# RockingMat/Prot2Text-V2-esm3

Measured on AMD Instinct MI355X. Metric: contrastive-step samples/sec (protein-text pairs), higher is better.
Workload: dtype bf16; 1 GPU; cfg3: esm2_t36_3B + Llama-3.1-8B-Instruct (text layers 1-16), per-GPU batch 16 x 1024 residues / 16 x 128 text tokens, readout mix, InfoNCE tau=0.05, adapter fwd+bwd + clip + AdamW, train mode (dropout 0.3), segments 1; global_batch=16, parallelism=dp1 (single process, no collective), streams=text tower and encoder segments on separate HIP streams

## Files before the change

### prot2text-v2-esm3_amd/csrc/epilogue.h

```cpp
#pragma once
#include "common.h"

namespace p2t {

struct EpiParams {
    const float* bias;
    void* out;
    void* z;
    int64_t ldc;
    int64_t M;
    int N;
    int n_zero;
    int accumulate;
    float drop_p;
    float drop_scale;
    uint64_t drop_seed;
    const float* cs;
    void* q; void* k; void* v;
    int seq, nh, nkv;
    int head_dim;
    float q_scale;
    const uint8_t* row_scale = nullptr;
};

// ... 30 lines not shown
        v[c] = t.x; v[c + 1] = t.y; v[c + 2] = t.z; v[c + 3] = t.w;
    }
}
template <int W> __device__ __forceinline__ void loadW(const bf16_t* p, float (&v)[W]) {
    if constexpr (W == 8) {
        load8(p, v);
    } else {
        load4(p, v);
    }
}
template <int W> __device__ __forceinline__ void zeroW(float (&v)[W]) {
#pragma unroll
    for (int c = 0; c < W; ++c) v[c] = 0.f;
}

#define P2T_EPI_APPLY2                                                                                          \
    template <int W, bool IN = false>                                                                           \
    __device__ __forceinline__ static void apply2(const EpiParams& p, int64_t m, int n, const float (&v0)[W],   \
                                                  const float (&v1)[W], const float (&b0)[W], const float (&b1)[W]) { \
        group<W, IN>(p, m, n, v0, b0);                                                                          \
        group<W, IN>(p, m, n + 32, v1, b1);                                                                     \
    }

template <typename Tout> constexpr int kStoreOps8 = (int)(8 * sizeof(Tout) / 16);

template <typename Tout>
struct EpiStore {
    static constexpr bool kRmw = false;
    static constexpr int kMinOps = 2 * kStoreOps8<Tout>;
    template <int W, bool IN = false>
    __device__ __forceinline__ static void group(const EpiParams& p, int64_t m, int n, const float (&v)[W], const float (&b)[W]) {
        Tout* o = (Tout*)p.out + m * p.ldc + n;
        float r[W];
        if (IN || n < p.N) {
#pragma unroll
            for (int j = 0; j < W; ++j) r[j] = v[j] + b[j];
            storeW<W>(o, r);
        } else if (n < p.n_zero) {
            zeroW<W>(r);
            storeW<W>(o, r);
        }
    }
    P2T_EPI_APPLY2
};

template <typename Tout, bool EXTRA = false>
struct EpiGelu {
    static constexpr bool kRmw = false;
    static constexpr int kMinOps = 2 * kStoreOps8<Tout>;
    template <int W, bool IN = false>
    __device__ __forceinline__ static void group(const EpiParams& p, int64_t m, int n, const float (&v)[W], const float (&b)[W]) {
        Tout* o = (Tout*)p.out + m * p.ldc + n;
        float zv[W], r[W];
        if (IN || n < p.N) {
#pragma unroll
            for (int j = 0; j < W; ++j) {
                zv[j] = v[j] + b[j];
                r[j] = gelu_erf_for<Tout>(zv[j]);
                if constexpr (EXTRA) {
                    if (p.drop_p > 0.f) r[j] = dropout_keep(p.drop_seed, m * (int64_t)p.N + n + j, p.drop_p) ? r[j] * p.drop_scale : 0.f;
                }
            }
            if constexpr (EXTRA) {
                if (p.z) storeW<W>((Tout*)p.z + m * p.ldc + n, zv);
            }
            storeW<W>(o, r);
        } else if (n < p.n_zero) {
            zeroW<W>(r);
            storeW<W>(o, r);
            if constexpr (EXTRA) {
                if (p.z) storeW<W>((Tout*)p.z + m * p.ldc + n, r);
            }
        }
    }
    P2T_EPI_APPLY2
};

__device__ __forceinline__ unsigned epi_pack_fp8x4(float a, float b, float c, float d) {
    int r = 0;
    r = __builtin_amdgcn_cvt_pk_fp8_f32(a, b, r, false);
    r = __builtin_amdgcn_cvt_pk_fp8_f32(c, d, r, true);
    return (unsigned)r;
}
struct EpiGeluFp8 {
    static constexpr bool kRmw = false;
    static constexpr int kMinOps = 2;
    template <int W, bool IN = false>
    __device__ __forceinline__ static void group(const EpiParams& p, int64_t m, int n, const float (&v)[W], const float (&b)[W]) {
        static_assert(W == 8, "fp8 output: MFMA kernels only (8 consecutive columns per lane)");
        uint8_t* o = (uint8_t*)p.out + m * p.ldc + n;
// ... 81 lines not shown
#pragma unroll
            for (int j = 0; j < W; ++j) r[j] += v[j];
        } else {
#pragma unroll
            for (int j = 0; j < W; ++j) r[j] = v[j];
        }
        storeW<W>(o, r);
    }
    P2T_EPI_APPLY2
};

template <typename Tout>
struct EpiSwiglu {
    static constexpr bool kRmw = false;
    static constexpr int kMinOps = kStoreOps8<Tout>;
    template <int W, bool IN = false>
    __device__ __forceinline__ static void apply2(const EpiParams& p, int64_t m, int n, const float (&g)[W], const float (&u)[W],
                                                  const float (&b0)[W], const float (&b1)[W]) {
        const int f = (n >> 6) * 32 + (n & 31);
        Tout* o = (Tout*)p.out + m * p.ldc + f;
        float r[W];
        if (IN || n < p.N) {
#pragma unroll
            for (int j = 0; j < W; ++j) r[j] = silu_for<Tout>(g[j]) * u[j];
            storeW<W>(o, r);
        } else if (f < p.n_zero) {
            zeroW<W>(r);
            storeW<W>(o, r);
        }
    }
};

template <typename Tout>
struct EpiQkvRope {
    static constexpr bool kRmw = false;
    static constexpr int kMinOps = 2 * kStoreOps8<Tout>;
    static constexpr bool kFetch = true;
    __device__ __forceinline__ static bool fetch_shared(const EpiParams& p) { return p.head_dim == 64; }
    template <int W, bool UNI = false>
    __device__ __forceinline__ static void fetch2(const EpiParams& p, int64_t m, int n, float (&c)[W], float (&s)[W]) {
        const int hd = p.head_dim, half = hd >> 1;
        const int blk = UNI ? __builtin_amdgcn_readfirstlane(n >> 6) : n >> 6;
        const int head = hd == 64 ? blk : blk >> 1;
        const int j = (hd == 64 ? 0 : 32 * (blk & 1)) + (n & 31);
        const uint32_t mu = (uint32_t)m, sq = (uint32_t)p.seq;
        const uint32_t b = mu / sq, t = mu - b * sq;
        if (UNI || head < p.nh + p.nkv) {
            loadW<W>(p.cs + (size_t)(t * (uint32_t)hd) + j, c);
            loadW<W>(p.cs + (size_t)(t * (uint32_t)hd) + half + j, s);
        }
    }
    template <int W, bool UNI = false>
    __device__ __forceinline__ static void apply2_fetched(const EpiParams& p, int64_t m, int n, const float (&v0)[W], const float (&v1)[W],
                                                          const float (&b0)[W], const float (&b1)[W], const float (&c)[W], const float (&s)[W]) {
        const int hd = p.head_dim, half = hd >> 1;
        const int blk = UNI ? __builtin_amdgcn_readfirstlane(n >> 6) : n >> 6;
        const int head = hd == 64 ? blk : blk >> 1;
        const int j = (hd == 64 ? 0 : 32 * (blk & 1)) + (n & 31);
        const uint32_t mu = (uint32_t)m, sq = (uint32_t)p.seq;
        const uint32_t b = mu / sq, t = mu - b * sq;
        float x1[W], x2[W];
#pragma unroll
        for (int e = 0; e < W; ++e) { x1[e] = v0[e] + b0[e]; x2[e] = v1[e] + b1[e]; }
        Tout* dst;
        if (head < p.nh + p.nkv) {
            const bool is_q = head < p.nh;
            const float sc = is_q ? p.q_scale : 1.0f;
            float o1[W], o2[W];
#pragma unroll
            for (int e = 0; e < W; ++e) {
                const float a1 = x1[e] * sc, a2 = x2[e] * sc;
                o1[e] = a1 * c[e] - a2 * s[e];
                o2[e] = a2 * c[e] + a1 * s[e];
            }
            dst = is_q ? (Tout*)p.q + (size_t)((b * (uint32_t)p.nh + (uint32_t)head) * sq + t) * (size_t)hd
                       : (Tout*)p.k + (size_t)((b * (uint32_t)p.nkv + (uint32_t)(head - p.nh)) * sq + t) * (size_t)hd;
            storeW<W>(dst + j, o1);
            storeW<W>(dst + half + j, o2);
        } else {
            dst = (Tout*)p.v + (size_t)((b * (uint32_t)p.nkv + (uint32_t)(head - p.nh - p.nkv)) * sq + t) * (size_t)hd;
            storeW<W>(dst + j, x1);
            storeW<W>(dst + half + j, x2);
        }
    }
    template <int W, bool IN = false>
    __device__ __forceinline__ static void apply2(const EpiParams& p, int64_t m, int n, const float (&v0)[W], const float (&v1)[W],
                                                  const float (&b0)[W], const float (&b1)[W]) {
        if (!IN && n >= p.N) return;
        float c[W], s[W];
#pragma unroll
        for (int e = 0; e < W; ++e) c[e] = s[e] = 0.f;
        fetch2<W>(p, m, n, c, s);
        apply2_fetched<W>(p, m, n, v0, v1, b0, b1, c, s);
    }
};

}
// ... 1 lines not shown
```

### prot2text-v2-esm3_amd/csrc/gemm_tile_common.h

```cpp
#pragma once
#include "common.h"
#include <type_traits>

#include "epilogue.h"

namespace p2t {

struct SplitFix {
    float* slab;
    unsigned* flag;
    unsigned* timeout;
    unsigned epoch;
};
enum { TILE_FULL = 0, TILE_PRODUCE = 1, TILE_CONSUME = 2 };


__device__ __forceinline__ void tile_coords(int id, int n_items, int tiles_m, int tiles_n, int& tm, int& tn) {
    const int q8 = n_items >> 3, r8 = n_items & 7, xcd = id & 7;
    const int swz_id = (xcd < r8 ? xcd * (q8 + 1) : r8 * (q8 + 1) + (xcd - r8) * q8) + (id >> 3);
    constexpr int GM = 4;
    const int band = swz_id / (GM * tiles_n), first_m = band * GM;
    const int gm = min(GM, tiles_m - first_m);
    const int in_band = swz_id - band * GM * tiles_n;
    tm = first_m + in_band % gm;
// ... 41 lines not shown
                v0[4] += p1.x + poison; v0[5] += p1.y + poison; v0[6] += p1.z + poison; v0[7] += p1.w + poison;
                v1[0] += p2.x + poison; v1[1] += p2.y + poison; v1[2] += p2.z + poison; v1[3] += p2.w + poison;
                v1[4] += p3.x + poison; v1[5] += p3.y + poison; v1[6] += p3.z + poison; v1[7] += p3.w + poison;
            }
            Epi::template apply2<8, INTERIOR>(ep, m, nb, v0, v1, b0, b1);
        }
    }
}

template <typename Epi, typename = void> struct epi_has_fetch_shared : std::false_type {};
template <typename Epi> struct epi_has_fetch_shared<Epi, std::void_t<decltype(&Epi::fetch_shared)>> : std::true_type {};
template <typename Epi, typename = void> struct epi_has_fetch : std::false_type {};
template <typename Epi> struct epi_has_fetch<Epi, std::void_t<decltype(Epi::kFetch)>> : std::true_type {};
#define P2T_EPI_PIN_GROUP(h, j) \
    asm volatile("" : "+a"(acc[h][0][j]), "+a"(acc[h][1][j]), "+a"(acc[h][2][j]), "+a"(acc[h][3][j])::"memory");
template <int MT, typename Epi, int P = 4>
__device__ __forceinline__ void tile_epilogue_pair(f32x4 (&acc)[2][4][MT], const EpiParams& ep, int64_t m0, int n0, int wm, int wn, int fr, int kg) {
    const int nb0 = n0 + wn * 128 + kg * 8;
    float b[2][2][8];
#pragma unroll
    for (int h = 0; h < 2; ++h)
#pragma unroll
        for (int e = 0; e < 8; ++e) b[h][0][e] = b[h][1][e] = 0.f;
    if (ep.bias) {
#pragma unroll
        for (int h = 0; h < 2; ++h) {
            loadW<8>(ep.bias + nb0 + h * 64, b[h][0]);
            loadW<8>(ep.bias + nb0 + h * 64 + 32, b[h][1]);
        }
    }
    const int64_t mrow = m0 + wm * MT * 16 + fr;
    if constexpr (epi_has_fetch_shared<Epi>::value && P > 0) {
// ... 8 lines not shown
            for (int u = 0; u < PS; ++u) Epi::template fetch2<8, true>(ep, mrow + u * 16, nb0, r[u][0], r[u][1]);
            __builtin_amdgcn_sched_barrier(0);
#pragma unroll
            for (int u = 0; u < MT; ++u) {
                float s0[8], s1[8];
#pragma unroll
                for (int e = 0; e < 8; ++e) { s0[e] = r[u % PS][0][e]; s1[e] = r[u % PS][1][e]; }
                __builtin_amdgcn_sched_barrier(0);
                if (u + PS < MT) Epi::template fetch2<8, true>(ep, mrow + (u + PS) * 16, nb0, r[u % PS][0], r[u % PS][1]);
                __builtin_amdgcn_sched_barrier(0);
#pragma unroll
                for (int h = 0; h < 2; ++h) {
                    P2T_EPI_PIN_GROUP(h, u)
                    const float v0[8] = {acc[h][0][u][0], acc[h][0][u][1], acc[h][0][u][2], acc[h][0][u][3], acc[h][1][u][0], acc[h][1][u][1], acc[h][1][u][2], acc[h][1][u][3]};
                    const float v1[8] = {acc[h][2][u][0], acc[h][2][u][1], acc[h][2][u][2], acc[h][2][u][3], acc[h][3][u][0], acc[h][3][u][1], acc[h][3][u][2], acc[h][3][u][3]};
                    Epi::template apply2_fetched<8, true>(ep, mrow + u * 16, nb0 + h * 64, v0, v1, b[h][0], b[h][1], s0, s1);
                    __builtin_amdgcn_sched_barrier(0);
                }
            }
            return;
        }
    }
    if constexpr ((Epi::kRmw || epi_has_fetch<Epi>::value) && P > 0) {
        constexpr int G = 2 * MT;
        float r[P][2][8];
        if constexpr (!Epi::kRmw) {
#pragma unroll
            for (int g = 0; g < P; ++g)
#pragma unroll
                for (int e = 0; e < 8; ++e) r[g][0][e] = r[g][1][e] = 0.f;
        }
// ... 11 lines not shown
            for (int e = 0; e < 8; ++e) { s0[e] = r[g % P][0][e]; s1[e] = r[g % P][1][e]; }
            __builtin_amdgcn_sched_barrier(0);
            if (g + P < G) Epi::template fetch2<8, true>(ep, mrow + ((g + P) % MT) * 16, nb0 + ((g + P) / MT) * 64, r[g % P][0], r[g % P][1]);
            __builtin_amdgcn_sched_barrier(0);
            Epi::template apply2_fetched<8, true>(ep, mrow + j * 16, nb0 + h * 64, v0, v1, b[h][0], b[h][1], s0, s1);
            __builtin_amdgcn_sched_barrier(0);
        }
    } else {
#pragma unroll
        for (int h = 0; h < 2; ++h)
#pragma unroll
            for (int j = 0; j < MT; ++j) {
                P2T_EPI_PIN_GROUP(h, j)
                const float v0[8] = {acc[h][0][j][0], acc[h][0][j][1], acc[h][0][j][2], acc[h][0][j][3], acc[h][1][j][0], acc[h][1][j][1], acc[h][1][j][2], acc[h][1][j][3]};
                const float v1[8] = {acc[h][2][j][0], acc[h][2][j][1], acc[h][2][j][2], acc[h][2][j][3], acc[h][3][j][0], acc[h][3][j][1], acc[h][3][j][2], acc[h][3][j][3]};
                Epi::template apply2<8, true>(ep, mrow + j * 16, nb0 + h * 64, v0, v1, b[h][0], b[h][1]);
                __builtin_amdgcn_sched_barrier(0);
            }
    }
}

}
```

### prot2text-v2-esm3_amd/csrc/gemm_w4.hip

```cpp
#include <type_traits>

#include "common.h"
#include "epilogue.h"
#include "gemm_tile_common.h"
#include "kernels.h"

namespace p2t {
#ifdef P2T_LAB
__device__ uint64_t* g_lab_stamp_ptr = nullptr;
#endif

typedef __bf16 bf16x8 __attribute__((ext_vector_type(8)));

template <typename Epi, bool PERSIST, int SCHED = 1, bool PAIRS_ONLY = false>
__global__ void __launch_bounds__(256)
    gemm_nt_w4_kernel(const bf16_t* __restrict__ A, int64_t lda, const bf16_t* __restrict__ W, int64_t ldw, int64_t M, int N, int K,
                      int tiles_m, int tiles_n, int n_items, int n_tail, int n_cover, EpiParams ep, SplitFix fix) {
    constexpr int MT = 8, NT = 8, BUF = 512 * 128, WOFF = 256 * 128, NL = 16;
#ifndef P2T_LAB
    static_assert(SCHED == 1, "the product library carries one instruction order of the K loop; order 0 is in the lab build");
#endif
    constexpr int kEpiOps = 2 * MT * Epi::kMinOps;
    constexpr int kIssuedBeforeWait = SCHED == 0 ? 6 : 9;
    constexpr int kExtCount = kIssuedBeforeWait + kEpiOps > 63 ? 63 : kIssuedBeforeWait + kEpiOps;
    __shared__ __attribute__((aligned(16))) char smem[2 * BUF];

    const int lane = threadIdx.x & 63;
    const int w = __builtin_amdgcn_readfirstlane(threadIdx.x >> 6);
    const int wm = w >> 1, wn = w & 1;
    const int nk = K >> 6;

    int item = blockIdx.x;
    int tm, tn;
    const int n_order = n_items + n_tail;
    tile_coords(item, n_order, tiles_m, tiles_n, tm, tn);
    int64_t m0 = (int64_t)tm * 256;
    int n0 = tn * 256;

    const char* a_ptr = (const char*)(A + m0 * lda);
// ... 34 lines not shown
        asm volatile("s_mov_b32 m0, %2\n\ts_nop 0\n\tglobal_load_lds_dwordx4 %0, %1" ::"v"(vo), "s"(sb), "s"(lds) : "memory");
    };
    auto mm_dma = [&](auto first, f32x4& c, const bf16x8& a, const bf16x8& b, int piece, int buf) {
        const char* sb = piece < 8 ? a_ptr : w_ptr;
        const uint32_t vo = piece < 8 ? a_voff[piece & 7] : w_voff[piece & 7];
        const uint32_t lds = lds0 + buf * BUF + (piece < 8 ? 0 : WOFF) + (w * 8 + (piece & 7)) * 1024;
        if constexpr (decltype(first)::value)
            asm volatile("s_mov_b32 m0, %5\n\tv_mfma_f32_16x16x32_bf16 %0, %1, %2, 0\n\tglobal_load_lds_dwordx4 %3, %4"
                         : "=a"(c) : "v"(a), "v"(b), "v"(vo), "s"(sb), "s"(lds) : "memory");
        else
            asm volatile("s_mov_b32 m0, %5\n\tv_mfma_f32_16x16x32_bf16 %0, %1, %2, %0\n\tglobal_load_lds_dwordx4 %3, %4"
                         : "+a"(c) : "v"(a), "v"(b), "v"(vo), "s"(sb), "s"(lds) : "memory");
    };
    using T = std::true_type;
    using F = std::false_type;
    auto stage = [&](f32x4 (&acc)[2][4][MT], auto bufc, auto first, auto rt, bool ext, bool more) {
        constexpr int B = decltype(bufc)::value;
        constexpr bool RT = decltype(rt)::value;
        using FI = decltype(first);
        const uint32_t xs1 = (x_addr + B * BUF) ^ 64u, ws1 = (w_addr + B * BUF) ^ 64u;
        const uint32_t xs0 = x_addr + (B ^ 1) * BUF, ws0 = w_addr + (B ^ 1) * BUF;
#define P2T_W4_PAIR(FF, WF, XF, P)                                                                            \
        mm(FF{}, acc[(((P) & 3) * 2) >> 2][(((P) & 3) * 2) & 3][(P) >> 2], WF[((P) & 3) * 2], XF[(P) >> 2]);   \
        mm(FF{}, acc[(((P) & 3) * 2 + 1) >> 2][(((P) & 3) * 2 + 1) & 3][(P) >> 2], WF[((P) & 3) * 2 + 1], XF[(P) >> 2]);
#define P2T_W4_R1W(I) rd(wb[I], ws1, std::integral_constant<int, (I) * 2048>{});
#define P2T_W4_R1X(J) rd(xb[J], xs1, std::integral_constant<int, (J) * 2048>{});
#define P2T_W4_R0W(I) rd(wa[I], ws0, std::integral_constant<int, (I) * 2048>{});
#define P2T_W4_R0X(J) rd(xa[J], xs0, std::integral_constant<int, (J) * 2048>{});
#define P2T_W4_G(Q) if (!RT || more) dma1(Q, B);
#define P2T_W4_GPAIR(Q, FF, WF, XF, P)                                                                                           \
        if constexpr (!RT) {                                                                                                     \
            mm_dma(FF{}, acc[(((P) & 3) * 2) >> 2][(((P) & 3) * 2) & 3][(P) >> 2], WF[((P) & 3) * 2], XF[(P) >> 2], Q, B);       \
            mm(FF{}, acc[(((P) & 3) * 2 + 1) >> 2][(((P) & 3) * 2 + 1) & 3][(P) >> 2], WF[((P) & 3) * 2 + 1], XF[(P) >> 2]);     \
        } else {                                                                                                                 \
            P2T_W4_G(Q) P2T_W4_PAIR(FF, WF, XF, P)                                                                               \
        }
#define P2T_W4_WAIT_NEXT_STAGE                                                                                                  \
        if (RT && !more) asm volatile("s_waitcnt vmcnt(0)\n\ts_barrier" ::: "memory");                                          \
        else if (FI::value && ext) asm volatile("s_waitcnt vmcnt(%0)\n\ts_barrier" ::"n"(kExtCount) : "memory");                 \
        else asm volatile("s_waitcnt vmcnt(%0)\n\ts_barrier" ::"n"(kIssuedBeforeWait) : "memory");
        if constexpr (SCHED == 1) {
            P2T_W4_R1W(0) P2T_W4_R1W(1) P2T_W4_PAIR(FI, wa, xa, 0) P2T_W4_R1X(0) P2T_W4_R1W(2) P2T_W4_PAIR(FI, wa, xa, 1) P2T_W4_R1W(3) P2T_W4_R1X(1) P2T_W4_PAIR(FI, wa, xa, 2) P2T_W4_R1W(4) P2T_W4_R1W(5) P2T_W4_PAIR(FI, wa, xa, 3)
            P2T_W4_R1X(2) P2T_W4_R1W(6) P2T_W4_PAIR(FI, wa, xa, 4) P2T_W4_R1W(7) P2T_W4_R1X(3) P2T_W4_PAIR(FI, wa, xa, 5) P2T_W4_R1X(4) P2T_W4_R1X(5) P2T_W4_PAIR(FI, wa, xa, 6) P2T_W4_R1X(6) P2T_W4_R1X(7) P2T_W4_PAIR(FI, wa, xa, 7)
            P2T_W4_PAIR(FI, wa, xa, 8) P2T_W4_PAIR(FI, wa, xa, 9) P2T_W4_PAIR(FI, wa, xa, 10)
            asm volatile("s_waitcnt lgkmcnt(0)\n\ts_barrier" ::: "memory");
            P2T_W4_GPAIR(0, FI, wa, xa, 11)
            P2T_W4_PAIR(FI, wa, xa, 12) P2T_W4_PAIR(FI, wa, xa, 13) P2T_W4_GPAIR(1, FI, wa, xa, 14) P2T_W4_PAIR(FI, wa, xa, 15)
            P2T_W4_PAIR(FI, wa, xa, 16) P2T_W4_GPAIR(2, FI, wa, xa, 17) P2T_W4_PAIR(FI, wa, xa, 18) P2T_W4_PAIR(FI, wa, xa, 19)
            P2T_W4_GPAIR(3, FI, wa, xa, 20) P2T_W4_PAIR(FI, wa, xa, 21) P2T_W4_PAIR(FI, wa, xa, 22) P2T_W4_GPAIR(4, FI, wa, xa, 23)
            P2T_W4_PAIR(FI, wa, xa, 24) P2T_W4_PAIR(FI, wa, xa, 25) P2T_W4_GPAIR(5, FI, wa, xa, 26) P2T_W4_PAIR(FI, wa, xa, 27)
            P2T_W4_PAIR(FI, wa, xa, 28) P2T_W4_GPAIR(6, FI, wa, xa, 29) P2T_W4_PAIR(FI, wa, xa, 30) P2T_W4_PAIR(FI, wa, xa, 31)
            P2T_W4_GPAIR(7, F, wb, xb, 0) P2T_W4_PAIR(F, wb, xb, 1) P2T_W4_PAIR(F, wb, xb, 2) P2T_W4_GPAIR(8, F, wb, xb, 3)
            P2T_W4_WAIT_NEXT_STAGE
            P2T_W4_R0W(0) P2T_W4_PAIR(F, wb, xb, 4) P2T_W4_R0W(1) P2T_W4_PAIR(F, wb, xb, 5) P2T_W4_R0X(0) P2T_W4_GPAIR(9, F, wb, xb, 6) P2T_W4_R0W(2) P2T_W4_PAIR(F, wb, xb, 7)
            P2T_W4_R0W(3) P2T_W4_PAIR(F, wb, xb, 8) P2T_W4_R0X(1) P2T_W4_GPAIR(10, F, wb, xb, 9) P2T_W4_R0W(4) P2T_W4_PAIR(F, wb, xb, 10) P2T_W4_R0W(5) P2T_W4_PAIR(F, wb, xb, 11)
            P2T_W4_R0X(2) P2T_W4_GPAIR(11, F, wb, xb, 12) P2T_W4_R0W(6) P2T_W4_PAIR(F, wb, xb, 13) P2T_W4_R0W(7) P2T_W4_PAIR(F, wb, xb, 14) P2T_W4_R0X(3) P2T_W4_GPAIR(12, F, wb, xb, 15)
            P2T_W4_R0X(4) P2T_W4_PAIR(F, wb, xb, 16) P2T_W4_R0X(5) P2T_W4_PAIR(F, wb, xb, 17) P2T_W4_R0X(6) P2T_W4_GPAIR(13, F, wb, xb, 18) P2T_W4_R0X(7) P2T_W4_PAIR(F, wb, xb, 19)
            P2T_W4_PAIR(F, wb, xb, 20) P2T_W4_GPAIR(14, F, wb, xb, 21) P2T_W4_PAIR(F, wb, xb, 22) P2T_W4_PAIR(F, wb, xb, 23)
            P2T_W4_GPAIR(15, F, wb, xb, 24) P2T_W4_PAIR(F, wb, xb, 25) P2T_W4_PAIR(F, wb, xb, 26) P2T_W4_PAIR(F, wb, xb, 27)
// ... 18 lines not shown
            P2T_W4_R0X(4) P2T_W4_GPAIR(10, F, wb, xb, 16) P2T_W4_R0X(5) P2T_W4_PAIR(F, wb, xb, 17) P2T_W4_R0X(6) P2T_W4_PAIR(F, wb, xb, 18) P2T_W4_R0X(7) P2T_W4_GPAIR(11, F, wb, xb, 19)
            P2T_W4_PAIR(F, wb, xb, 20) P2T_W4_PAIR(F, wb, xb, 21) P2T_W4_GPAIR(12, F, wb, xb, 22) P2T_W4_PAIR(F, wb, xb, 23)
            P2T_W4_PAIR(F, wb, xb, 24) P2T_W4_GPAIR(13, F, wb, xb, 25) P2T_W4_PAIR(F, wb, xb, 26) P2T_W4_PAIR(F, wb, xb, 27)
            P2T_W4_GPAIR(14, F, wb, xb, 28) P2T_W4_PAIR(F, wb, xb, 29) P2T_W4_PAIR(F, wb, xb, 30) P2T_W4_GPAIR(15, F, wb, xb, 31)
        }
#endif
        a_ptr += 128; w_ptr += 128;
#undef P2T_W4_WAIT_NEXT_STAGE
#undef P2T_W4_PAIR
#undef P2T_W4_R1W
#undef P2T_W4_R1X
#undef P2T_W4_R0W
#undef P2T_W4_R0X
#undef P2T_W4_G
#undef P2T_W4_GPAIR
        asm volatile("s_waitcnt lgkmcnt(0)" ::: "memory");
    };
    using I0 = std::integral_constant<int, 0>;
    using I1 = std::integral_constant<int, 1>;

    auto prologue = [&]() {
#pragma unroll
    for (int b = 0; b < 2; ++b) {
#pragma unroll
        for (int q = 0; q < NL; ++q) dma1(q, b);
        a_ptr += 128; w_ptr += 128;
    }
    asm volatile("s_waitcnt vmcnt(%0)\n\ts_barrier" ::"n"(NL) : "memory");
    rd(wa[0], w_addr, std::integral_constant<int, 0>{}); rd(wa[1], w_addr, std::integral_constant<int, 2048>{});
    rd(wa[2], w_addr, std::integral_constant<int, 4096>{}); rd(wa[3], w_addr, std::integral_constant<int, 6144>{});
    rd(wa[4], w_addr, std::integral_constant<int, 8192>{}); rd(wa[5], w_addr, std::integral_constant<int, 10240>{});
    rd(wa[6], w_addr, std::integral_constant<int, 12288>{}); rd(wa[7], w_addr, std::integral_constant<int, 14336>{});
    rd(xa[0], x_addr, std::integral_constant<int, 0>{}); rd(xa[1], x_addr, std::integral_constant<int, 2048>{});
    rd(xa[2], x_addr, std::integral_constant<int, 4096>{}); rd(xa[3], x_addr, std::integral_constant<int, 6144>{});
    rd(xa[4], x_addr, std::integral_constant<int, 8192>{}); rd(xa[5], x_addr, std::integral_constant<int, 10240>{});
    rd(xa[6], x_addr, std::integral_constant<int, 12288>{}); rd(xa[7], x_addr, std::integral_constant<int, 14336>{});
    asm volatile("s_waitcnt lgkmcnt(0)" ::: "memory");
    };
    auto k_loop = [&](f32x4 (&acc)[2][4][MT], int nk_l, bool ext, bool has_next, int64_t nm0, int nn0) {
        stage(acc, I0{}, T{}, F{}, ext, true);
        stage(acc, I1{}, F{}, F{}, false, true);
        for (int s = 2; s + 2 < nk_l; s += 2) {
            stage(acc, I0{}, F{}, F{}, false, true);
            stage(acc, I1{}, F{}, F{}, false, true);
        }
        if (has_next) {
            a_ptr = (const char*)(A + nm0 * lda);
            w_ptr = (const char*)(W + (int64_t)nn0 * ldw);
        }
        stage(acc, I0{}, F{}, T{}, false, has_next);
        stage(acc, I1{}, F{}, T{}, false, has_next);
        asm volatile("s_nop 7\n\ts_nop 7\n\ts_nop 7" ::: "memory");
#pragma unroll
        for (int h = 0; h < 2; ++h)
#pragma unroll
            for (int i = 0; i < 4; ++i)
#pragma unroll
                for (int j = 0; j < MT; ++j) asm volatile("" : "+a"(acc[h][i][j]));
    };
    if constexpr (!PAIRS_ONLY) {
    prologue();
    {
        f32x4 acc[2][4][MT];
        bool ext = false;
#ifdef P2T_LAB
        constexpr bool kDiagEpi = std::is_same<Epi, EpiStore<bf16_t>>::value || std::is_same<Epi, EpiGelu<bf16_t, false>>::value || std::is_same<Epi, EpiResid>::value;
        uint64_t* dbgp = kDiagEpi ? (uint64_t*)ep.z : nullptr;
        if (!dbgp) dbgp = g_lab_stamp_ptr;
        const bool diag = PERSIST && dbgp != nullptr;
        uint64_t d_loop = 0, d_epi = 0, d_gap = 0, d_tiles = 0, d_real = 0, t_end = 0;
        auto now = [&]() -> uint64_t { uint64_t t; asm volatile("s_memtime %0\n\ts_waitcnt lgkmcnt(0)" : "=s"(t)::"memory"); return t; };
        auto now_real = [&]() -> uint64_t { uint64_t t; asm volatile("s_memrealtime %0\n\ts_waitcnt lgkmcnt(0)" : "=s"(t)::"memory"); return t; };
#endif
        for (;;) {
            const int nxt = item + (int)gridDim.x;
            const bool has_next = PERSIST && nxt < n_items;
            int64_t nm0 = 0;
            int nn0 = 0;
            if (has_next) {
                tile_coords(nxt, n_order, tiles_m, tiles_n, tm, tn);
                nm0 = (int64_t)tm * 256;
                nn0 = tn * 256;
            }
#ifdef P2T_LAB
            uint64_t t0 = 0, r0 = 0, t1 = 0;
            if (diag) { t0 = now(); r0 = now_real(); if (ext) d_gap += t0 - t_end; }
#endif
            k_loop(acc, nk, ext, has_next, nm0, nn0);
#ifdef P2T_LAB
            if (diag) { t1 = now(); d_loop += t1 - t0; d_real += now_real() - r0; d_tiles += 1; }
#endif
            if (PERSIST) {
                int fr_e = fr, kg_e = kg;
                asm volatile("" : "+v"(fr_e), "+v"(kg_e));
                tile_epilogue_pair<MT, Epi, (epi_has_fetch<Epi>::value && !Epi::kRmw) ? 2 : 4>(acc, ep, m0, n0, wm, wn, fr_e, kg_e);
            } else {
                const bool interior = m0 + 256 <= M && n0 + 256 <= N && n0 + 256 <= n_cover;
                if (interior) {
                    tile_epilogue<MT, Epi, true>(acc[0], ep, M, N, n_cover, m0, n0, wm, 2 * wn, fr, kg);
                    tile_epilogue<MT, Epi, true>(acc[1], ep, M, N, n_cover, m0, n0, wm, 2 * wn + 1, fr, kg);
                } else {
                    tile_epilogue<MT, Epi, false>(acc[0], ep, M, N, n_cover, m0, n0, wm, 2 * wn, fr, kg);
                    tile_epilogue<MT, Epi, false>(acc[1], ep, M, N, n_cover, m0, n0, wm, 2 * wn + 1, fr, kg);
                }
            }
#ifdef P2T_LAB
            if (diag) {
                t_end = now();
                d_epi += t_end - t1;
                if (!has_next && threadIdx.x == 0) {
                    uint64_t* d = dbgp + (size_t)blockIdx.x * 8;
                    d[0] = d_loop; d[1] = d_epi; d[2] = d_gap; d[3] = d_tiles; d[4] = d_real;
                }
            }
#endif
            if (!has_next) break;
            ext = true;
            item = nxt;
            m0 = nm0;
            n0 = nn0;
        }
    }
    }
    if (PERSIST && (int)blockIdx.x < 2 * n_tail) {
        const bool producer = (int)blockIdx.x < n_tail;
        const int t = producer ? (int)blockIdx.x : (int)blockIdx.x - n_tail;
        const int nk0 = (nk >> 1) & ~1;
        tile_coords(n_items + t, n_order, tiles_m, tiles_n, tm, tn);
        m0 = (int64_t)tm * 256;
        n0 = tn * 256;
        a_ptr = (const char*)(A + m0 * lda + (producer ? nk0 * 64 : 0));
        w_ptr = (const char*)(W + (int64_t)n0 * ldw + (producer ? nk0 * 64 : 0));
        asm volatile("s_waitcnt vmcnt(0) lgkmcnt(0)\n\ts_barrier" ::: "memory");
        prologue();
        f32x4 acc2[2][4][MT];
        k_loop(acc2, producer ? nk - nk0 : nk0, false, false, 0, 0);
        if (producer) {
            float4* slab = reinterpret_cast<float4*>(fix.slab) + (int64_t)t * (64 * 256) + threadIdx.x;
#pragma unroll
            for (int h = 0; h < 2; ++h)
#pragma unroll
                for (int i = 0; i < 4; ++i)
#pragma unroll
                    for (int j = 0; j < MT; ++j)
                        slab[((h * 4 + i) * MT + j) * 256] = make_float4(acc2[h][i][j][0], acc2[h][i][j][1], acc2[h][i][j][2], acc2[h][i][j][3]);
            asm volatile("s_waitcnt vmcnt(0)" ::: "memory");
            __syncthreads();
            if (w == 0) {
                __builtin_amdgcn_fence(__ATOMIC_RELEASE, "agent");
                asm volatile("s_waitcnt vmcnt(0)" ::: "memory");
                __hip_atomic_store(fix.flag + t, fix.epoch, __ATOMIC_RELAXED, __HIP_MEMORY_SCOPE_AGENT);
// ... 41 lines not shown
    return P2T_OK;
}

template <typename Epi>
int launch_gemm_w4_persist(const void* A, int64_t lda, const void* W, int64_t ldw, int64_t M, int N, int K, int n_items, int n_tail, int grid,
                           const EpiParams& ep, const SplitFix& fix, hipStream_t s, int sched) {
    const dim3 g((unsigned)(grid < n_items ? grid : n_items));
#ifdef P2T_LAB
    if (sched == 0) {
        gemm_nt_w4_kernel<Epi, true, 0><<<g, 256, 0, s>>>((const bf16_t*)A, lda, (const bf16_t*)W, ldw, M, N, K, (int)(M / 256), N / 256, n_items, n_tail, N, ep, fix);
        P2T_LAUNCH_CHECK();
        return P2T_OK;
    }
#endif
    P2T_REQUIRE(sched == 1, "gemm (four-wave): instruction order %d is not in this build", sched);
    gemm_nt_w4_kernel<Epi, true, 1><<<g, 256, 0, s>>>((const bf16_t*)A, lda, (const bf16_t*)W, ldw, M, N, K, (int)(M / 256), N / 256, n_items, n_tail, N, ep, fix);
    P2T_LAUNCH_CHECK();
    return P2T_OK;
}
template <typename Epi>
int launch_gemm_w4_pairs(const void* A, int64_t lda, const void* W, int64_t ldw, int64_t M, int N, int K, int n_tail, const EpiParams& ep,
                         const SplitFix& fix, hipStream_t s) {
    gemm_nt_w4_kernel<Epi, true, 1, true><<<dim3((unsigned)(2 * n_tail)), 256, 0, s>>>((const bf16_t*)A, lda, (const bf16_t*)W, ldw, M, N, K, (int)(M / 256),
                                                                                      N / 256, 0, n_tail, N, ep, fix);
    P2T_LAUNCH_CHECK();
    return P2T_OK;
}
template int launch_gemm_w4_pairs<EpiResid>(const void*, int64_t, const void*, int64_t, int64_t, int, int, int, const EpiParams&, const SplitFix&, hipStream_t);
template int launch_gemm_w4_pairs<EpiStore<bf16_t>>(const void*, int64_t, const void*, int64_t, int64_t, int, int, int, const EpiParams&, const SplitFix&, hipStream_t);
template int launch_gemm_w4_pairs<EpiStore<float>>(const void*, int64_t, const void*, int64_t, int64_t, int, int, int, const EpiParams&, const SplitFix&, hipStream_t);
// ... 10 lines not shown
    if (K % 128 != 0 || K < 256 || M < 1 || (int64_t)256 * (lda > ldw ? lda : ldw) * 2 >= (int64_t)1 << 32) return P2T_ERR_UNSUPPORTED;
    const bool ob = out_dtype == P2T_BF16;
    switch (epilogue) {
        case P2T_EPI_STORE: return ob ? launch_w4<EpiStore<bf16_t>>(A, lda, W, ldw, M, N, K, n_cover, ep, s) : launch_w4<EpiStore<float>>(A, lda, W, ldw, M, N, K, n_cover, ep, s);
        case P2T_EPI_GELU: if (ob) return launch_w4<EpiGelu<bf16_t>>(A, lda, W, ldw, M, N, K, n_cover, ep, s); break;
        case P2T_EPI_RESID: return launch_w4<EpiResid>(A, lda, W, ldw, M, N, K, n_cover, ep, s);
        case P2T_EPI_QKV_ROPE: if (ob) return launch_w4<EpiQkvRope<bf16_t>>(A, lda, W, ldw, M, N, K, n_cover, ep, s); break;
        default: break;
    }
    return P2T_ERR_UNSUPPORTED;
}

}

#ifdef P2T_LAB
extern "C" int p2t_lab_set_stamp_buffer(void* ptr) {
    uint64_t* p = (uint64_t*)ptr;
    return (int)hipMemcpyToSymbol(HIP_SYMBOL(p2t::g_lab_stamp_ptr), &p, sizeof(p));
}
#endif
```

Before: 172.4 samples/s.

## Defer half of persistent w4 GEMM epilogue stores into next tile's k-loop

In the persistent four-wave GEMM, the second half of each tile's epilogue bf16 stores is packed into registers instead of being written immediately. Those stores are then issued interleaved with MFMA pairs during the first four stages of the next tile's k-loop, with adjusted vmcnt waits. The aim is to hide epilogue store latency behind the next tile's compute rather than stalling between tiles. The cost is extra register pressure for the parked data and addresses, plus more complex wait-count bookkeeping. It is enabled only when there are more tiles than the grid and K is deep enough.

```diff
diff --git a/prot2text-v2-esm3_amd/csrc/epilogue.h b/prot2text-v2-esm3_amd/csrc/epilogue.h
--- a/prot2text-v2-esm3_amd/csrc/epilogue.h
+++ b/prot2text-v2-esm3_amd/csrc/epilogue.h
@@ -68,6 +68,22 @@
     for (int c = 0; c < W; ++c) v[c] = 0.f;
 }
 
+struct EpiStoreNow {
+    template <int W, typename T> __device__ __forceinline__ void put(T* p, const float (&v)[W]) { storeW<W>(p, v); }
+};
+struct EpiParkSink {
+    p2t_u32x4* data;
+    const void** addr;
+    int n = 0;
+    template <int W> __device__ __forceinline__ void put(bf16_t* p, const float (&v)[W]) {
+        static_assert(W == 8, "parked stores are 16-byte bf16 stores");
+        data[n] = p2t_u32x4{pack_bf16x2(v[0], v[1]), pack_bf16x2(v[2], v[3]), pack_bf16x2(v[4], v[5]), pack_bf16x2(v[6], v[7])};
+        addr[n] = p;
+        ++n;
+    }
+    template <int W> __device__ __forceinline__ void put(float*, const float (&)[W]) { static_assert(W < 0, "only bf16 outputs are parked"); }
+};
+
 #define P2T_EPI_APPLY2                                                                                          \
     template <int W, bool IN = false>                                                                           \
     __device__ __forceinline__ static void apply2(const EpiParams& p, int64_t m, int n, const float (&v0)[W],   \
@@ -76,34 +92,46 @@
         group<W, IN>(p, m, n + 32, v1, b1);                                                                     \
     }
 
+#define P2T_EPI_APPLY2_SINK                                                                                     \
+    template <int W, bool IN = false, typename St = EpiStoreNow>                                                \
+    __device__ __forceinline__ static void apply2(const EpiParams& p, int64_t m, int n, const float (&v0)[W],   \
+                                                  const float (&v1)[W], const float (&b0)[W], const float (&b1)[W], St&& st = St{}) { \
+        group<W, IN>(p, m, n, v0, b0, st);                                                                      \
+        group<W, IN>(p, m, n + 32, v1, b1, st);                                                                 \
+    }
+
 template <typename Tout> constexpr int kStoreOps8 = (int)(8 * sizeof(Tout) / 16);
 
 template <typename Tout>
 struct EpiStore {
     static constexpr bool kRmw = false;
     static constexpr int kMinOps = 2 * kStoreOps8<Tout>;
-    template <int W, bool IN = false>
-    __device__ __forceinline__ static void group(const EpiParams& p, int64_t m, int n, const float (&v)[W], const float (&b)[W]) {
+    static constexpr int kPark = sizeof(Tout) == 2 ? 2 : 0;
+    __device__ __forceinline__ static int64_t park_row_bytes(const EpiParams& p) { return p.ldc * (int64_t)(16 * sizeof(Tout)); }
+    template <int W, bool IN = false, typename St = EpiStoreNow>
+    __device__ __forceinline__ static void group(const EpiParams& p, int64_t m, int n, const float (&v)[W], const float (&b)[W], St&& st = St{}) {
         Tout* o = (Tout*)p.out + m * p.ldc + n;
         float r[W];
         if (IN || n < p.N) {
 #pragma unroll
             for (int j = 0; j < W; ++j) r[j] = v[j] + b[j];
-            storeW<W>(o, r);
+            st.template put<W>(o, r);
         } else if (n < p.n_zero) {
             zeroW<W>(r);
             storeW<W>(o, r);
         }
     }
-    P2T_EPI_APPLY2
+    P2T_EPI_APPLY2_SINK
 };
 
 template <typename Tout, bool EXTRA = false>
 struct EpiGelu {
     static constexpr bool kRmw = false;
     static constexpr int kMinOps = 2 * kStoreOps8<Tout>;
-    template <int W, bool IN = false>
-    __device__ __forceinline__ static void group(const EpiParams& p, int64_t m, int n, const float (&v)[W], const float (&b)[W]) {
+    static constexpr int kPark = (sizeof(Tout) == 2 && !EXTRA) ? 2 : 0;
+    __device__ __forceinline__ static int64_t park_row_bytes(const EpiParams& p) { return p.ldc * (int64_t)(16 * sizeof(Tout)); }
+    template <int W, bool IN = false, typename St = EpiStoreNow>
+    __device__ __forceinline__ static void group(const EpiParams& p, int64_t m, int n, const float (&v)[W], const float (&b)[W], St&& st = St{}) {
         Tout* o = (Tout*)p.out + m * p.ldc + n;
         float zv[W], r[W];
         if (IN || n < p.N) {
@@ -118,7 +146,7 @@
             if constexpr (EXTRA) {
                 if (p.z) storeW<W>((Tout*)p.z + m * p.ldc + n, zv);
             }
-            storeW<W>(o, r);
+            st.template put<W>(o, r);
         } else if (n < p.n_zero) {
             zeroW<W>(r);
             storeW<W>(o, r);
@@ -127,7 +155,7 @@
             }
         }
     }
-    P2T_EPI_APPLY2
+    P2T_EPI_APPLY2_SINK
 };
 
 __device__ __forceinline__ unsigned epi_pack_fp8x4(float a, float b, float c, float d) {
@@ -239,16 +267,18 @@
 struct EpiSwiglu {
     static constexpr bool kRmw = false;
     static constexpr int kMinOps = kStoreOps8<Tout>;
-    template <int W, bool IN = false>
+    static constexpr int kPark = sizeof(Tout) == 2 ? 1 : 0;
+    __device__ __forceinline__ static int64_t park_row_bytes(const EpiParams& p) { return p.ldc * (int64_t)(16 * sizeof(Tout)); }
+    template <int W, bool IN = false, typename St = EpiStoreNow>
     __device__ __forceinline__ static void apply2(const EpiParams& p, int64_t m, int n, const float (&g)[W], const float (&u)[W],
-                                                  const float (&b0)[W], const float (&b1)[W]) {
+                                                  const float (&b0)[W], const float (&b1)[W], St&& st = St{}) {
         const int f = (n >> 6) * 32 + (n & 31);
         Tout* o = (Tout*)p.out + m * p.ldc + f;
         float r[W];
         if (IN || n < p.N) {
 #pragma unroll
             for (int j = 0; j < W; ++j) r[j] = silu_for<Tout>(g[j]) * u[j];
-            storeW<W>(o, r);
+            st.template put<W>(o, r);
         } else if (f < p.n_zero) {
             zeroW<W>(r);
             storeW<W>(o, r);
@@ -261,6 +291,8 @@
     static constexpr bool kRmw = false;
     static constexpr int kMinOps = 2 * kStoreOps8<Tout>;
     static constexpr bool kFetch = true;
+    static constexpr int kPark = 0;
+    __device__ __forceinline__ static int64_t park_row_bytes(const EpiParams& p) { return (int64_t)p.head_dim * (int64_t)(16 * sizeof(Tout)); }
     __device__ __forceinline__ static bool fetch_shared(const EpiParams& p) { return p.head_dim == 64; }
     template <int W, bool UNI = false>
     __device__ __forceinline__ static void fetch2(const EpiParams& p, int64_t m, int n, float (&c)[W], float (&s)[W]) {
@@ -275,9 +307,10 @@
             loadW<W>(p.cs + (size_t)(t * (uint32_t)hd) + half + j, s);
         }
     }
-    template <int W, bool UNI = false>
+    template <int W, bool UNI = false, typename St = EpiStoreNow>
     __device__ __forceinline__ static void apply2_fetched(const EpiParams& p, int64_t m, int n, const float (&v0)[W], const float (&v1)[W],
-                                                          const float (&b0)[W], const float (&b1)[W], const float (&c)[W], const float (&s)[W]) {
+                                                          const float (&b0)[W], const float (&b1)[W], const float (&c)[W], const float (&s)[W],
+                                                          St&& st = St{}) {
         const int hd = p.head_dim, half = hd >> 1;
         const int blk = UNI ? __builtin_amdgcn_readfirstlane(n >> 6) : n >> 6;
         const int head = hd == 64 ? blk : blk >> 1;
@@ -300,12 +333,12 @@
             }
             dst = is_q ? (Tout*)p.q + (size_t)((b * (uint32_t)p.nh + (uint32_t)head) * sq + t) * (size_t)hd
                        : (Tout*)p.k + (size_t)((b * (uint32_t)p.nkv + (uint32_t)(head - p.nh)) * sq + t) * (size_t)hd;
-            storeW<W>(dst + j, o1);
-            storeW<W>(dst + half + j, o2);
+            st.template put<W>(dst + j, o1);
+            st.template put<W>(dst + half + j, o2);
         } else {
             dst = (Tout*)p.v + (size_t)((b * (uint32_t)p.nkv + (uint32_t)(head - p.nh - p.nkv)) * sq + t) * (size_t)hd;
-            storeW<W>(dst + j, x1);
-            storeW<W>(dst + half + j, x2);
+            st.template put<W>(dst + j, x1);
+            st.template put<W>(dst + half + j, x2);
         }
     }
     template <int W, bool IN = false>
diff --git a/prot2text-v2-esm3_amd/csrc/gemm_tile_common.h b/prot2text-v2-esm3_amd/csrc/gemm_tile_common.h
--- a/prot2text-v2-esm3_amd/csrc/gemm_tile_common.h
+++ b/prot2text-v2-esm3_amd/csrc/gemm_tile_common.h
@@ -79,8 +79,27 @@
 template <typename Epi> struct epi_has_fetch<Epi, std::void_t<decltype(Epi::kFetch)>> : std::true_type {};
 #define P2T_EPI_PIN_GROUP(h, j) \
     asm volatile("" : "+a"(acc[h][0][j]), "+a"(acc[h][1][j]), "+a"(acc[h][2][j]), "+a"(acc[h][3][j])::"memory");
-template <int MT, typename Epi, int P = 4>
-__device__ __forceinline__ void tile_epilogue_pair(f32x4 (&acc)[2][4][MT], const EpiParams& ep, int64_t m0, int n0, int wm, int wn, int fr, int kg) {
+template <int NS> struct W4Park {
+    p2t_u32x4 d[NS];
+    const void* a0;
+};
+template <int MT, typename Epi, int P = 4, typename PK = std::nullptr_t>
+__device__ __forceinline__ void tile_epilogue_pair(f32x4 (&acc)[2][4][MT], const EpiParams& ep, int64_t m0, int n0, int wm, int wn, int fr, int kg,
+                                                   PK* pk = nullptr) {
+    constexpr bool PARK = !std::is_same<PK, std::nullptr_t>::value;
+    auto emit = [&](int h, int j, auto&& fn) {
+        if constexpr (PARK) {
+            if (h == 1) {
+                const void* a[2];
+                EpiParkSink sk{&pk->d[j * Epi::kPark], a};
+                fn(sk);
+                if (j == 0) pk->a0 = a[0];
+                return;
+            }
+        }
+        EpiStoreNow now;
+        fn(now);
+    };
     const int nb0 = n0 + wn * 128 + kg * 8;
     float b[2][2][8];
 #pragma unroll
@@ -119,7 +138,8 @@
                     P2T_EPI_PIN_GROUP(h, u)
                     const float v0[8] = {acc[h][0][u][0], acc[h][0][u][1], acc[h][0][u][2], acc[h][0][u][3], acc[h][1][u][0], acc[h][1][u][1], acc[h][1][u][2], acc[h][1][u][3]};
                     const float v1[8] = {acc[h][2][u][0], acc[h][2][u][1], acc[h][2][u][2], acc[h][2][u][3], acc[h][3][u][0], acc[h][3][u][1], acc[h][3][u][2], acc[h][3][u][3]};
-                    Epi::template apply2_fetched<8, true>(ep, mrow + u * 16, nb0 + h * 64, v0, v1, b[h][0], b[h][1], s0, s1);
+                    if constexpr (PARK) emit(h, u, [&](auto& st) { Epi::template apply2_fetched<8, true>(ep, mrow + u * 16, nb0 + h * 64, v0, v1, b[h][0], b[h][1], s0, s1, st); });
+                    else Epi::template apply2_fetched<8, true>(ep, mrow + u * 16, nb0 + h * 64, v0, v1, b[h][0], b[h][1], s0, s1);
                     __builtin_amdgcn_sched_barrier(0);
                 }
             }
@@ -161,7 +181,8 @@
                 P2T_EPI_PIN_GROUP(h, j)
                 const float v0[8] = {acc[h][0][j][0], acc[h][0][j][1], acc[h][0][j][2], acc[h][0][j][3], acc[h][1][j][0], acc[h][1][j][1], acc[h][1][j][2], acc[h][1][j][3]};
                 const float v1[8] = {acc[h][2][j][0], acc[h][2][j][1], acc[h][2][j][2], acc[h][2][j][3], acc[h][3][j][0], acc[h][3][j][1], acc[h][3][j][2], acc[h][3][j][3]};
-                Epi::template apply2<8, true>(ep, mrow + j * 16, nb0 + h * 64, v0, v1, b[h][0], b[h][1]);
+                if constexpr (PARK) emit(h, j, [&](auto& st) { Epi::template apply2<8, true>(ep, mrow + j * 16, nb0 + h * 64, v0, v1, b[h][0], b[h][1], st); });
+                else Epi::template apply2<8, true>(ep, mrow + j * 16, nb0 + h * 64, v0, v1, b[h][0], b[h][1]);
                 __builtin_amdgcn_sched_barrier(0);
             }
     }
diff --git a/prot2text-v2-esm3_amd/csrc/gemm_w4.hip b/prot2text-v2-esm3_amd/csrc/gemm_w4.hip
--- a/prot2text-v2-esm3_amd/csrc/gemm_w4.hip
+++ b/prot2text-v2-esm3_amd/csrc/gemm_w4.hip
@@ -12,7 +12,28 @@
 
 typedef __bf16 bf16x8 __attribute__((ext_vector_type(8)));
 
-template <typename Epi, bool PERSIST, int SCHED = 1, bool PAIRS_ONLY = false>
+constexpr int kDrainPerStage = 4, kDrainBeforeWait = 4;
+constexpr int kW4MaxParked = 16;
+constexpr int kW4DrainStages = (kW4MaxParked + kDrainPerStage - 1) / kDrainPerStage;
+constexpr int kW4DeferMinStages = kW4DrainStages + 2;
+constexpr int w4_drain_wait(int d, int parked, int epi_ops, int before) {
+    int left = parked - d * kDrainPerStage;
+    left = left < 0 ? 0 : left > kDrainPerStage ? kDrainPerStage : left;
+    const int c = before + (left < kDrainBeforeWait ? left : kDrainBeforeWait) + (d == 0 ? epi_ops : 0);
+    return c > 63 ? 63 : c;
+}
+template <typename Epi, typename = void> struct epi_park : std::integral_constant<int, 0> {};
+template <typename Epi> struct epi_park<Epi, std::void_t<decltype(Epi::kPark)>> : std::integral_constant<int, Epi::kPark> {};
+#ifdef P2T_STORE_PLAIN
+#define P2T_W4_NT ""
+#else
+#define P2T_W4_NT " nt"
+#endif
+#ifdef P2T_LAB
+static bool g_lab_w4_defer = true;
+#endif
+
+template <typename Epi, bool PERSIST, int SCHED = 1, bool PAIRS_ONLY = false, bool DEFER = false>
 __global__ void __launch_bounds__(256)
     gemm_nt_w4_kernel(const bf16_t* __restrict__ A, int64_t lda, const bf16_t* __restrict__ W, int64_t ldw, int64_t M, int N, int K,
                       int tiles_m, int tiles_n, int n_items, int n_tail, int n_cover, EpiParams ep, SplitFix fix) {
@@ -23,6 +44,15 @@
     constexpr int kEpiOps = 2 * MT * Epi::kMinOps;
     constexpr int kIssuedBeforeWait = SCHED == 0 ? 6 : 9;
     constexpr int kExtCount = kIssuedBeforeWait + kEpiOps > 63 ? 63 : kIssuedBeforeWait + kEpiOps;
+    static_assert(!DEFER || (PERSIST && !PAIRS_ONLY && SCHED == 1 && epi_park<Epi>::value > 0), "deferred stores: persistent form, order 1, a functor that parks");
+    constexpr int kPark = epi_park<Epi>::value;
+    constexpr int NS = DEFER ? MT * kPark : 1;
+    constexpr int kEpiOpsNow = MT * Epi::kMinOps;
+    static_assert(NS <= kW4MaxParked, "parked stores");
+    W4Park<NS> pk;
+    uint32_t park_voff = 0;
+    const char* park_base = nullptr;
+    int64_t park_rowb = 0;
     __shared__ __attribute__((aligned(16))) char smem[2 * BUF];
 
     const int lane = threadIdx.x & 63;
@@ -87,8 +117,14 @@
     };
     using T = std::true_type;
     using F = std::false_type;
-    auto stage = [&](f32x4 (&acc)[2][4][MT], auto bufc, auto first, auto rt, bool ext, bool more) {
+    auto pst = [](auto cc, uint32_t voff, const p2t_u32x4& d, const char* rb) {
+        asm volatile("global_store_dwordx4 %0, %1, %2 offset:%3" P2T_W4_NT ::"v"(voff), "v"(d), "s"(rb), "n"(decltype(cc)::value * 64) : "memory");
+    };
+    constexpr int kParkDiv = kPark > 0 ? kPark : 1;
+    auto stage = [&](f32x4 (&acc)[2][4][MT], auto bufc, auto first, auto rt, auto dsc, bool ext, bool more) {
         constexpr int B = decltype(bufc)::value;
+        constexpr int DS = decltype(dsc)::value;
+        constexpr int kDrainCount = w4_drain_wait(DS < 0 ? 0 : DS, NS, kEpiOpsNow, kIssuedBeforeWait);
         constexpr bool RT = decltype(rt)::value;
         using FI = decltype(first);
         const uint32_t xs1 = (x_addr + B * BUF) ^ 64u, ws1 = (w_addr + B * BUF) ^ 64u;
@@ -108,14 +144,24 @@
         } else {                                                                                                                 \
             P2T_W4_G(Q) P2T_W4_PAIR(FF, WF, XF, P)                                                                               \
         }
+#define P2T_W4_SPAIR(KK, FF, WF, XF, P)                                                                                          \
+        if constexpr (DS >= 0 && DS * kDrainPerStage + (KK) < NS) {                                                              \
+            mm(FF{}, acc[(((P) & 3) * 2) >> 2][(((P) & 3) * 2) & 3][(P) >> 2], WF[((P) & 3) * 2], XF[(P) >> 2]);                 \
+            if (ext) pst(std::integral_constant<int, (DS * kDrainPerStage + (KK)) % kParkDiv>{}, park_voff, pk.d[DS * kDrainPerStage + (KK)],    \
+                         park_base + ((DS * kDrainPerStage + (KK)) / kParkDiv) * park_rowb);                                       \
+            mm(FF{}, acc[(((P) & 3) * 2 + 1) >> 2][(((P) & 3) * 2 + 1) & 3][(P) >> 2], WF[((P) & 3) * 2 + 1], XF[(P) >> 2]);     \
+        } else {                                                                                                                 \
+            P2T_W4_PAIR(FF, WF, XF, P)                                                                                           \
+        }
 #define P2T_W4_WAIT_NEXT_STAGE                                                                                                  \
         if (RT && !more) asm volatile("s_waitcnt vmcnt(0)\n\ts_barrier" ::: "memory");                                          \
-        else if (FI::value && ext) asm volatile("s_waitcnt vmcnt(%0)\n\ts_barrier" ::"n"(kExtCount) : "memory");                 \
+        else if (DS >= 0 && ext) asm volatile("s_waitcnt vmcnt(%0)\n\ts_barrier" ::"n"(kDrainCount) : "memory");                 \
+        else if (DS < 0 && FI::value && ext) asm volatile("s_waitcnt vmcnt(%0)\n\ts_barrier" ::"n"(kExtCount) : "memory");                 \
         else asm volatile("s_waitcnt vmcnt(%0)\n\ts_barrier" ::"n"(kIssuedBeforeWait) : "memory");
         if constexpr (SCHED == 1) {
-            P2T_W4_R1W(0) P2T_W4_R1W(1) P2T_W4_PAIR(FI, wa, xa, 0) P2T_W4_R1X(0) P2T_W4_R1W(2) P2T_W4_PAIR(FI, wa, xa, 1) P2T_W4_R1W(3) P2T_W4_R1X(1) P2T_W4_PAIR(FI, wa, xa, 2) P2T_W4_R1W(4) P2T_W4_R1W(5) P2T_W4_PAIR(FI, wa, xa, 3)
-            P2T_W4_R1X(2) P2T_W4_R1W(6) P2T_W4_PAIR(FI, wa, xa, 4) P2T_W4_R1W(7) P2T_W4_R1X(3) P2T_W4_PAIR(FI, wa, xa, 5) P2T_W4_R1X(4) P2T_W4_R1X(5) P2T_W4_PAIR(FI, wa, xa, 6) P2T_W4_R1X(6) P2T_W4_R1X(7) P2T_W4_PAIR(FI, wa, xa, 7)
-            P2T_W4_PAIR(FI, wa, xa, 8) P2T_W4_PAIR(FI, wa, xa, 9) P2T_W4_PAIR(FI, wa, xa, 10)
+            P2T_W4_R1W(0) P2T_W4_R1W(1) P2T_W4_PAIR(FI, wa, xa, 0) P2T_W4_R1X(0) P2T_W4_R1W(2) P2T_W4_SPAIR(0, FI, wa, xa, 1) P2T_W4_R1W(3) P2T_W4_R1X(1) P2T_W4_PAIR(FI, wa, xa, 2) P2T_W4_R1W(4) P2T_W4_R1W(5) P2T_W4_PAIR(FI, wa, xa, 3)
+            P2T_W4_R1X(2) P2T_W4_R1W(6) P2T_W4_SPAIR(1, FI, wa, xa, 4) P2T_W4_R1W(7) P2T_W4_R1X(3) P2T_W4_PAIR(FI, wa, xa, 5) P2T_W4_R1X(4) P2T_W4_R1X(5) P2T_W4_PAIR(FI, wa, xa, 6) P2T_W4_R1X(6) P2T_W4_R1X(7) P2T_W4_SPAIR(2, FI, wa, xa, 7)
+            P2T_W4_PAIR(FI, wa, xa, 8) P2T_W4_SPAIR(3, FI, wa, xa, 9) P2T_W4_PAIR(FI, wa, xa, 10)
             asm volatile("s_waitcnt lgkmcnt(0)\n\ts_barrier" ::: "memory");
             P2T_W4_GPAIR(0, FI, wa, xa, 11)
             P2T_W4_PAIR(FI, wa, xa, 12) P2T_W4_PAIR(FI, wa, xa, 13) P2T_W4_GPAIR(1, FI, wa, xa, 14) P2T_W4_PAIR(FI, wa, xa, 15)
@@ -164,10 +210,12 @@
 #undef P2T_W4_R0X
 #undef P2T_W4_G
 #undef P2T_W4_GPAIR
+#undef P2T_W4_SPAIR
         asm volatile("s_waitcnt lgkmcnt(0)" ::: "memory");
     };
     using I0 = std::integral_constant<int, 0>;
     using I1 = std::integral_constant<int, 1>;
+    using DN = std::integral_constant<int, -1>;
 
     auto prologue = [&]() {
 #pragma unroll
@@ -187,19 +235,36 @@
     rd(xa[6], x_addr, std::integral_constant<int, 12288>{}); rd(xa[7], x_addr, std::integral_constant<int, 14336>{});
     asm volatile("s_waitcnt lgkmcnt(0)" ::: "memory");
     };
-    auto k_loop = [&](f32x4 (&acc)[2][4][MT], int nk_l, bool ext, bool has_next, int64_t nm0, int nn0) {
-        stage(acc, I0{}, T{}, F{}, ext, true);
-        stage(acc, I1{}, F{}, F{}, false, true);
-        for (int s = 2; s + 2 < nk_l; s += 2) {
-            stage(acc, I0{}, F{}, F{}, false, true);
-            stage(acc, I1{}, F{}, F{}, false, true);
+#ifdef P2T_LAB
+    uint64_t* lab_drain_end = nullptr;
+#endif
+    auto k_loop = [&](auto drainc, f32x4 (&acc)[2][4][MT], int nk_l, bool ext, bool has_next, int64_t nm0, int nn0) {
+        constexpr bool DRAIN = decltype(drainc)::value;
+        int s = 2;
+        if constexpr (DRAIN) {
+            static_assert(kW4DrainStages == 4, "the peeled drain stages below");
+            stage(acc, I0{}, T{}, F{}, std::integral_constant<int, 0>{}, ext, true);
+            stage(acc, I1{}, F{}, F{}, std::integral_constant<int, 1>{}, ext, true);
+            stage(acc, I0{}, F{}, F{}, std::integral_constant<int, 2>{}, ext, true);
+            stage(acc, I1{}, F{}, F{}, std::integral_constant<int, 3>{}, ext, true);
+            s = 4;
+#ifdef P2T_LAB
+            if (lab_drain_end) { uint64_t t; asm volatile("s_memtime %0\n\ts_waitcnt lgkmcnt(0)" : "=s"(t)::"memory"); *lab_drain_end = t; }
+#endif
+        } else {
+            stage(acc, I0{}, T{}, F{}, DN{}, ext, true);
+            stage(acc, I1{}, F{}, F{}, DN{}, false, true);
+        }
+        for (; s + 2 < nk_l; s += 2) {
+            stage(acc, I0{}, F{}, F{}, DN{}, false, true);
+            stage(acc, I1{}, F{}, F{}, DN{}, false, true);
         }
         if (has_next) {
             a_ptr = (const char*)(A + nm0 * lda);
             w_ptr = (const char*)(W + (int64_t)nn0 * ldw);
         }
-        stage(acc, I0{}, F{}, T{}, false, has_next);
-        stage(acc, I1{}, F{}, T{}, false, has_next);
+        stage(acc, I0{}, F{}, T{}, DN{}, false, has_next);
+        stage(acc, I1{}, F{}, T{}, DN{}, false, has_next);
         asm volatile("s_nop 7\n\ts_nop 7\n\ts_nop 7" ::: "memory");
 #pragma unroll
         for (int h = 0; h < 2; ++h)
@@ -218,7 +283,8 @@
         uint64_t* dbgp = kDiagEpi ? (uint64_t*)ep.z : nullptr;
         if (!dbgp) dbgp = g_lab_stamp_ptr;
         const bool diag = PERSIST && dbgp != nullptr;
-        uint64_t d_loop = 0, d_epi = 0, d_gap = 0, d_tiles = 0, d_real = 0, t_end = 0;
+        uint64_t d_loop = 0, d_epi = 0, d_gap = 0, d_tiles = 0, d_real = 0, t_end = 0, d_drain = 0, d_drained = 0, d_first = 0, t_drain = 0;
+        if (diag && DEFER) lab_drain_end = &t_drain;
         auto now = [&]() -> uint64_t { uint64_t t; asm volatile("s_memtime %0\n\ts_waitcnt lgkmcnt(0)" : "=s"(t)::"memory"); return t; };
         auto now_real = [&]() -> uint64_t { uint64_t t; asm volatile("s_memrealtime %0\n\ts_waitcnt lgkmcnt(0)" : "=s"(t)::"memory"); return t; };
 #endif
@@ -236,14 +302,30 @@
             uint64_t t0 = 0, r0 = 0, t1 = 0;
             if (diag) { t0 = now(); r0 = now_real(); if (ext) d_gap += t0 - t_end; }
 #endif
-            k_loop(acc, nk, ext, has_next, nm0, nn0);
-#ifdef P2T_LAB
-            if (diag) { t1 = now(); d_loop += t1 - t0; d_real += now_real() - r0; d_tiles += 1; }
+            k_loop(std::integral_constant<bool, DEFER>{}, acc, nk, ext, has_next, nm0, nn0);
+#ifdef P2T_LAB
+            if (diag) {
+                t1 = now(); d_loop += t1 - t0; d_real += now_real() - r0; d_tiles += 1;
+                if (DEFER) { if (ext) { d_drain += t_drain - t0; d_drained += 1; } else d_first += t_drain - t0; }
+            }
 #endif
             if (PERSIST) {
                 int fr_e = fr, kg_e = kg;
                 asm volatile("" : "+v"(fr_e), "+v"(kg_e));
-                tile_epilogue_pair<MT, Epi, (epi_has_fetch<Epi>::value && !Epi::kRmw) ? 2 : 4>(acc, ep, m0, n0, wm, wn, fr_e, kg_e);
+                constexpr int kAhead = (epi_has_fetch<Epi>::value && !Epi::kRmw) ? 2 : 4;
+                bool parked = false;
+                if constexpr (DEFER) {
+                    if (has_next) {
+                        tile_epilogue_pair<MT, Epi, kAhead, W4Park<NS>>(acc, ep, m0, n0, wm, wn, fr_e, kg_e, &pk);
+                        const uint64_t a0 = (uint64_t)pk.a0;
+                        const uint64_t b0 = ((uint64_t)(uint32_t)__builtin_amdgcn_readfirstlane((int)(a0 >> 32)) << 32) | (uint32_t)__builtin_amdgcn_readfirstlane((int)(uint32_t)a0);
+                        park_base = (const char*)b0;
+                        park_voff = (uint32_t)(a0 - b0);
+                        park_rowb = Epi::park_row_bytes(ep);
+                        parked = true;
+                    }
+                }
+                if (!parked) tile_epilogue_pair<MT, Epi, kAhead>(acc, ep, m0, n0, wm, wn, fr_e, kg_e);
             } else {
                 const bool interior = m0 + 256 <= M && n0 + 256 <= N && n0 + 256 <= n_cover;
                 if (interior) {
@@ -260,7 +342,7 @@
                 d_epi += t_end - t1;
                 if (!has_next && threadIdx.x == 0) {
                     uint64_t* d = dbgp + (size_t)blockIdx.x * 8;
-                    d[0] = d_loop; d[1] = d_epi; d[2] = d_gap; d[3] = d_tiles; d[4] = d_real;
+                    d[0] = d_loop; d[1] = d_epi; d[2] = d_gap; d[3] = d_tiles; d[4] = d_real; d[5] = d_drain; d[6] = d_drained; d[7] = d_first;
                 }
             }
 #endif
@@ -284,7 +366,7 @@
         asm volatile("s_waitcnt vmcnt(0) lgkmcnt(0)\n\ts_barrier" ::: "memory");
         prologue();
         f32x4 acc2[2][4][MT];
-        k_loop(acc2, producer ? nk - nk0 : nk0, false, false, 0, 0);
+        k_loop(F{}, acc2, producer ? nk - nk0 : nk0, false, false, 0, 0);
         if (producer) {
             float4* slab = reinterpret_cast<float4*>(fix.slab) + (int64_t)t * (64 * 256) + threadIdx.x;
 #pragma unroll
@@ -356,6 +438,18 @@
     }
 #endif
     P2T_REQUIRE(sched == 1, "gemm (four-wave): instruction order %d is not in this build", sched);
+    if constexpr (epi_park<Epi>::value > 0) {
+        bool defer = n_items > (int)g.x && K / 64 >= kW4DeferMinStages;
+        if constexpr (epi_has_fetch<Epi>::value) defer = defer && ep.head_dim == 64 && ep.seq % 128 == 0;
+#ifdef P2T_LAB
+        defer = defer && g_lab_w4_defer;
+#endif
+        if (defer) {
+            gemm_nt_w4_kernel<Epi, true, 1, false, true><<<g, 256, 0, s>>>((const bf16_t*)A, lda, (const bf16_t*)W, ldw, M, N, K, (int)(M / 256), N / 256, n_items, n_tail, N, ep, fix);
+            P2T_LAUNCH_CHECK();
+            return P2T_OK;
+        }
+    }
     gemm_nt_w4_kernel<Epi, true, 1><<<g, 256, 0, s>>>((const bf16_t*)A, lda, (const bf16_t*)W, ldw, M, N, K, (int)(M / 256), N / 256, n_items, n_tail, N, ep, fix);
     P2T_LAUNCH_CHECK();
     return P2T_OK;
@@ -396,6 +490,10 @@
 }
 
 #ifdef P2T_LAB
+extern "C" int p2t_lab_set_w4_defer(int on) {
+    p2t::g_lab_w4_defer = on != 0;
+    return 0;
+}
 extern "C" int p2t_lab_set_stamp_buffer(void* ptr) {
     uint64_t* p = (uint64_t*)ptr;
     return (int)hipMemcpyToSymbol(HIP_SYMBOL(p2t::g_lab_stamp_ptr), &p, sizeof(p));
```

Result: no change. 171.8 samples/s (-0.4%).
